# nihalsid/single-view-3d-reconstruction

Measured on AMD Instinct MI355X. Metric: query-points/sec fwd+bwd (128^3 grid, 50k pts), higher is better.
Workload: dtype f32

## Files before the change

### include/svr_hip.h

```cpp
#ifndef SVR_HIP_H
#define SVR_HIP_H

#include <stdint.h>

#ifdef __cplusplus
extern "C" {
#endif

#define SVR_OK 0
#define SVR_E_BADARG (-1)
#define SVR_E_BADSHAPE (-2)
#define SVR_E_ALIGN (-3)
#define SVR_E_UNSUPPORTED (-4)
#define SVR_E_IO (-5)
#define SVR_E_NOTFOUND (-6)
#define SVR_E_INTERNAL (-7)

#define SVR_MAX_LEVELS 6

int svr_version(void);
const char *svr_last_error(void);

typedef struct svr_pull_plan {
  const uint32_t *keys;
// ... 138 lines not shown
#define SVR_LIN_FWD_F16X3 1
#define SVR_LIN_FWD_BF16X6 2
#define SVR_LIN_BWD_DATA_F32 3
#define SVR_LIN_BWD_DATA_F16X3S 4
#define SVR_LIN_BWD_DATA_BF16X3 5
#define SVR_LIN_BWD_WEIGHT_F32 6
#define SVR_LIN_BWD_WEIGHT_F16X3S 7
#define SVR_LIN_BWD_WEIGHT_BF16X3 8
#define SVR_LIN_K_NT 0
#define SVR_LIN_K_NN 1
#define SVR_LIN_K_TN 2
#define SVR_LIN_K_NT128 3
#define SVR_LIN_K_NT64 4
#define SVR_LIN_K_NT128_BWD 5
#define SVR_LIN_K_NN_X3 6
#define SVR_LIN_K_TN_TR 7
#define SVR_LIN_K_TN_PREPASS 8
#define SVR_LIN_K_NT_X6 9
#define SVR_LIN_BIAS_NONE 0
#define SVR_LIN_BIAS_KERNEL 1
#define SVR_LIN_BIAS_COLSUM_VEC 2
#define SVR_LIN_BIAS_COLSUM_SLOW 3
int svr_linear_variant(int32_t op, int64_t M, int64_t N, int64_t K, int64_t ld_a, int64_t ld_b, int64_t ld_out,
                       int64_t ld_mask, int32_t lo_a, int32_t lo_b, int32_t lo_out, int32_t lo_mask, int32_t epilogue,
                       int32_t want_bias, int32_t *kernel, int32_t *coalesced, int32_t *splits, int64_t *rows_per_split,
                       int32_t *bias_form, int32_t *status);

int svr_fc_out_fwd(const float *H, int64_t ldh, const float *w, const float *b, float *logits,
                   const int32_t *row_map, int64_t M, int64_t K, void *stream);
int64_t svr_fc_out_bwd_workspace(int64_t M, int64_t K);
int svr_fc_out_bwd(const float *H, int64_t ldh, const float *w, const float *dlogits,
                   const int32_t *row_map, float *dH, int64_t lddh, float *dw, float *db, int64_t M,
                   int64_t K, uint32_t *amax_dh, void *workspace, void *stream);

int svr_bce_logits_sum_mean(const float *logits, const float *targets, float *loss, float *dlogits,
                            int64_t B, int64_t N, float gscale, void *workspace, void *stream);
int64_t svr_bce_ordered_workspace(int64_t B);
int svr_bce_logits_sum_mean_ordered(const float *logits, const float *targets, float *loss, float *dlogits,
                                    int64_t B, int64_t N, float gscale, void *workspace, void *stream);

int svr_conv3d_pack_weight(const float *W , float *Wp_fwd, float *Wp_bwd,
                           int32_t Ci, int32_t Co, void *stream);
int svr_conv3d_unpack_wgrad(const float *dWp , float *dW ,
                            int32_t Ci, int32_t Co, void *stream);
int svr_conv3d_k3(const float *in, const float *Wp, const float *bias, float *out, int32_t B,
                  int32_t D, int32_t H, int32_t W, int32_t Ci, int32_t Co, int epilogue,
                  const float *mask, void *stream);
int64_t svr_conv3d_c1_fwd_stats_workspace(int32_t B, int32_t D, int32_t H, int32_t W, int32_t Co);
int svr_conv3d_c1_fwd_stats(const float *in, const float *Wp, const float *bias, float *out, double *stats,
                            int32_t B, int32_t D, int32_t H, int32_t W, int32_t Co, int epilogue,
                            void *workspace, void *stream);
int64_t svr_conv3d_fwd_bf16x6_workspace(int32_t Ci, int32_t Co);
int svr_conv3d_k3_fwd_bf16x6(const float *in, const float *W, const float *bias, float *out, int32_t B,
                             int32_t D, int32_t H, int32_t Wd, int32_t Ci, int32_t Co, int epilogue,
                             void *workspace, void *stream);
int64_t svr_conv3d_fwd_f16x3_workspace(int32_t Ci, int32_t Co);
int svr_conv3d_k3_fwd_f16x3(const float *in, const float *W, const float *bias, float *out, int32_t B,
                             int32_t D, int32_t H, int32_t Wd, int32_t Ci, int32_t Co, int epilogue,
                             void *workspace, void *stream);
int32_t svr_conv3d_fwd_f16x3_stats_blocks(int32_t B, int32_t D, int32_t H, int32_t Wd, int32_t Ci, int32_t Co);
int svr_conv3d_k3_fwd_f16x3_stats(const float *in, const float *W, const float *bias, float *out, double *part, int32_t B,
                                  int32_t D, int32_t H, int32_t Wd, int32_t Ci, int32_t Co, int epilogue,
                                  void *workspace, void *stream);
int64_t svr_conv3d_bwd_data_bf16x3_workspace(int32_t Ci, int32_t Co);
int svr_conv3d_k3_bwd_data_bf16x3(const float *dout, const float *W, float *din, int32_t B, int32_t D,
                                  int32_t H, int32_t Wd, int32_t Ci, int32_t Co, int epilogue,
// ... 295 lines not shown
```

### single-view-3d-reconstruction_amd/_lib.py

```python
import ctypes as C
import os

import numpy as np
import torch

_HERE = os.path.dirname(os.path.abspath(__file__))
LIB_PATH = os.path.join(_HERE, "lib", "libsvr_hip.so")

SVR_MAX_LEVELS = 6
EPI_NONE, EPI_BIAS, EPI_BIAS_RELU, EPI_MASK = 0, 1, 2, 3

P = C.c_void_p
I32, I64, F32 = C.c_int32, C.c_int64, C.c_float


class Conv2dDesc(C.Structure):
    _fields_ = [("src0", P), ("src1", P), ("B", I32), ("H", I32), ("W", I32), ("C0", I32), ("C1", I32), ("k", I32),
                ("stride", I32), ("act", I32), ("upsample", I32)]


class PullPlan(C.Structure):
    _fields_ = [("keys", P), ("recs", P), ("heads", P), ("n_items", I64)]


# ... 32 lines not shown
    "svr_gather_trilinear_fwd": (C.c_int, [C.POINTER(GatherDesc), P, P, P]),
    "svr_gather_fc0_supported": (C.c_int32, [C.POINTER(GatherDesc)]),
    "svr_gather_fc0_workspace": (C.c_int64, [C.POINTER(GatherDesc), I32]),
    "svr_gather_fc0_fwd": (C.c_int, [C.POINTER(GatherDesc), P, P, I64, P, P, I64, I32, P, I64, P, C.c_uint32, I32, P, P]),
    "svr_gather_fc0_prepare": (C.c_int, [C.POINTER(GatherDesc), P, I64, I32, P, I64, P, C.c_uint32, P, P]),
    "svr_gather_fc0_run": (C.c_int, [C.POINTER(GatherDesc), P, P, P, I64, I32, P, I64, P, C.c_uint32, I32, P, P]),
    "svr_gather_fc0_bf16_prepare": (C.c_int, [C.POINTER(GatherDesc), P, I64, I32, P, P]),
    "svr_gather_fc0_bf16_run": (C.c_int, [C.POINTER(GatherDesc), P, P, P, I64, I32, I32, P, P]),
    "svr_gather_trilinear_bwd": (C.c_int, [C.POINTER(GatherDesc), P, P, P, P]),
    "svr_gather_corner_indices": (C.c_int, [C.POINTER(GatherDesc), I32, P, P, P]),
    "svr_cast_f32_to_bf16": (C.c_int, [P, P, I64, P]),
    "svr_gather_trilinear_fwd_bf16": (C.c_int, [C.POINTER(GatherDesc), P, P, P]),
    "svr_linear_fwd_bf16": (C.c_int, [P, I64, P, I64, P, P, I64, I64, I64, I64, C.c_int, P]),
    "svr_fc_out_fwd_bf16": (C.c_int, [P, I64, P, P, P, P, I64, I64, P]),
    "svr_linear_fwd": (C.c_int, [P, I64, P, I64, P, P, I64, I64, I64, I64, C.c_int, P, I64, P]),
    "svr_linear_bwd_data": (C.c_int, [P, I64, P, I64, P, I64, I64, I64, I64, C.c_int, P, I64, P]),
    "svr_linear_bwd_weight_workspace": (I64, [I64, I64, I64]),
    "svr_linear_bwd_weight": (C.c_int, [P, I64, P, I64, P, I64, P, I64, I64, I64, P, P]),
    "svr_linear_fwd_bf16x6_workspace": (I64, [I64, I64]),
    "svr_linear_fwd_bf16x6": (C.c_int, [P, I64, P, I64, P, P, I64, I64, I64, I64, C.c_int, P, P]),
    "svr_linear_fwd_f16x3_workspace": (I64, [I64, I64]),
    "svr_linear_fwd_f16x3": (C.c_int, [P, I64, P, I64, P, P, I64, I64, I64, I64, C.c_int, P, P]),
    "svr_linear_bwd_data_bf16x3_workspace": (I64, [I64, I64]),
    "svr_linear_bwd_data_bf16x3": (C.c_int, [P, I64, P, I64, P, I64, I64, I64, I64, C.c_int, P, I64, P, P]),
    "svr_linear_bwd_weight_bf16x3_workspace": (I64, [I64, I64, I64]),
    "svr_linear_bwd_weight_bf16x3": (C.c_int, [P, I64, P, I64, P, I64, P, I64, I64, I64, P, P]),
    "svr_amax_f32": (C.c_int, [P, I64, I64, I64, P, P]),
    "svr_linear_bwd_data_f16x3_workspace": (I64, [I64, I64]),
    "svr_linear_bwd_data_f16x3": (C.c_int, [P, I64, P, I64, P, I64, I64, I64, I64, C.c_int, P, I64, P, P, P, P]),
    "svr_linear_bwd_weight_f16x3_workspace": (I64, [I64, I64, I64]),
    "svr_linear_bwd_weight_f16x3": (C.c_int, [P, I64, P, I64, P, I64, P, I64, I64, I64, P, P, P]),
    "svr_linear_variant": (C.c_int, [I32, I64, I64, I64, I64, I64, I64, I64, I32, I32, I32, I32, I32, I32, P, P, P, P, P, P]),
    "svr_fc_out_fwd": (C.c_int, [P, I64, P, P, P, P, I64, I64, P]),
    "svr_fc_out_bwd_workspace": (I64, [I64, I64]),
    "svr_fc_out_bwd": (C.c_int, [P, I64, P, P, P, P, I64, P, P, I64, I64, P, P, P]),
    "svr_bce_logits_sum_mean": (C.c_int, [P, P, P, P, I64, I64, F32, P, P]),
    "svr_bce_ordered_workspace": (I64, [I64]),
    "svr_bce_logits_sum_mean_ordered": (C.c_int, [P, P, P, P, I64, I64, F32, P, P]),
    "svr_conv3d_pack_weight": (C.c_int, [P, P, P, I32, I32, P]),
    "svr_conv3d_unpack_wgrad": (C.c_int, [P, P, I32, I32, P]),
    "svr_conv3d_k3": (C.c_int, [P, P, P, P, I32, I32, I32, I32, I32, I32, C.c_int, P, P]),
    "svr_conv3d_fwd_bf16x6_workspace": (I64, [I32, I32]),
    "svr_conv3d_k3_fwd_bf16x6": (C.c_int, [P, P, P, P, I32, I32, I32, I32, I32, I32, C.c_int, P, P]),
    "svr_conv3d_fwd_f16x3_workspace": (I64, [I32, I32]),
    "svr_conv3d_k3_fwd_f16x3": (C.c_int, [P, P, P, P, I32, I32, I32, I32, I32, I32, C.c_int, P, P]),
    "svr_conv3d_fwd_f16x3_stats_blocks": (I32, [I32, I32, I32, I32, I32, I32]),
    "svr_conv3d_k3_fwd_f16x3_stats": (C.c_int, [P, P, P, P, P, I32, I32, I32, I32, I32, I32, C.c_int, P, P]),
    "svr_conv3d_bwd_data_bf16x3_workspace": (I64, [I32, I32]),
    "svr_conv3d_k3_bwd_data_bf16x3": (C.c_int, [P, P, P, I32, I32, I32, I32, I32, I32, C.c_int, P, P, P]),
    "svr_conv3d_c1_fwd_stats_workspace": (I64, [I32, I32, I32, I32, I32]),
    "svr_conv3d_c1_fwd_stats": (C.c_int, [P, P, P, P, P, I32, I32, I32, I32, I32, C.c_int, P, P]),
    "svr_conv3d_k3_bwd_weight_workspace": (I64, [I32, I32, I32, I32, I32, I32]),
    "svr_conv3d_k3_bwd_weight": (C.c_int, [P, P, P, P, I32, I32, I32, I32, I32, I32, P, P]),
    "svr_conv3d_k3_bwd_weight_bf16x3_workspace": (I64, [I32, I32, I32, I32, I32, I32]),
    "svr_conv3d_k3_bwd_weight_bf16x3": (C.c_int, [P, P, P, P, I32, I32, I32, I32, I32, I32, P, P]),
    "svr_conv3d_k3_bwd_weight_bf16x3_param": (C.c_int, [P, P, P, P, I32, I32, I32, I32, I32, I32, P, P]),
    "svr_conv3d_bwd_data_f16x3_workspace": (I64, [I32, I32]),
    "svr_conv3d_k3_bwd_data_f16x3": (C.c_int, [P, P, P, I32, I32, I32, I32, I32, I32, C.c_int, P, P, P, P, P]),
    "svr_conv3d_k3_bwd_weight_f16x3": (C.c_int, [P, P, P, P, I32, I32, I32, I32, I32, I32, I32, P, P, P]),
    "svr_conv3d_k3_variant": (C.c_int, [I32, I32, I32, I32, I32, I32, I32, P, P, P, P, P]),
    "svr_conv3d_k3_bwd_weight_variant": (C.c_int, [I32, I32, I32, I32, I32, I32, I32, P, P, P]),
    "svr_bn_stats_workspace": (I64, [I64, I32]),
    "svr_bn_stats": (C.c_int, [P, P, I64, I32, P, P]),
    "svr_bn_stats_finalize": (C.c_int, [P, P, P, P, P, P, P, P, P, I64, I32, F32, F32, P, P]),
    "svr_bn_finalize_parts": (C.c_int, [P, I32, P, P, P, P, P, P, P, P, I64, I32, F32, F32, P]),
    "svr_bn_finalize": (C.c_int, [P, P, P, P, P, P, P, I64, I32, F32, F32, C.c_int, P]),
# ... 169 lines not shown
```

### single-view-3d-reconstruction_amd/build.py

```python
import os
import subprocess
import sys

HERE = os.path.dirname(os.path.abspath(__file__))
CSRC = os.path.join(HERE, "csrc")
INCLUDE = os.path.join(os.path.dirname(HERE), "include")
LIBDIR = os.path.join(HERE, "lib")
LIB = os.path.join(LIBDIR, "libsvr_hip.so")

SOURCES = {
    "capi.cpp": [],
    "gather.hip": ["-ffp-contract=off"],
    "gather_fc0.hip": ["-ffp-contract=off"],
    "sort.hip": [],
    "gemm.hip": [],
    "gemm_bf16x3.hip": [],
    "gemm_bf16x6.hip": [],
    "gemm_f16x3.hip": [],
    "conv3d.hip": [],
    "conv3d_bf16.hip": [],
    "conv3d_bwdw_bf16.hip": [],
    "bn_pool.hip": [],
    "stage1.hip": [],
    "projection.hip": ["-ffp-contract=off"],
    "bf16_path.hip": ["-ffp-contract=off"],
    "mesh_occupancy.hip": ["-ffp-contract=off"],
    "marching_cubes.hip": ["-ffp-contract=off"],
    "sparse_lattice.hip": ["-ffp-contract=off"],
    "voxel_mesh.hip": ["-ffp-contract=off"],
    "mesh_eval.hip": ["-ffp-contract=off"],
    "mesh_df.hip": ["-ffp-contract=off"],
    "raycast.hip": ["-ffp-contract=off"],
    "vertex_color.hip": ["-ffp-contract=off"],
    "mesh_components.hip": ["-ffp-contract=off"],
    "mesh_simplify.hip": ["-ffp-contract=off"],
    "mesh_smooth.hip": ["-ffp-contract=off"],
    "sample_io.hip": [],
    "io_npz.cpp": [],
    "io_df.cpp": [],
    "io_exr.cpp": [],
    "io_mesh.cpp": [],
    "io_png.cpp": [],
    "raw_sample.hip": ["-ffp-contract=off"],
    "conv2d.hip": [],
    "conv2d_igemm.hip": [],
    "depth_head.hip": ["-ffp-contract=off"],
    "rgb_preprocess.hip": ["-ffp-contract=off"],
}
HOST = ("capi.cpp", "io_npz.cpp", "io_df.cpp", "io_exr.cpp", "io_mesh.cpp", "io_png.cpp")
HOST_COMMON = ["-O3", "-fPIC", "-std=c++17", "-ffp-contract=off", "-I" + INCLUDE, "-I" + CSRC]
COMMON = ["-O3", "-fPIC", "--offload-arch=gfx950", "-munsafe-fp-atomics", "-std=c++17", "-I" + INCLUDE, "-I" + CSRC,
# ... 83 lines not shown
```

### single-view-3d-reconstruction_amd/model/ifnet.py

```python
import contextlib
import copy
import os

import torch
import torch.nn as nn

from .. import ops
from ..arena import StepArena

_ARCH = {
    128: dict(stages=[(("conv_in",), "conv_in_bn"), (("conv_0", "conv_0_1"), "conv0_1_bn"),
                      (("conv_1", "conv_1_1"), "conv1_1_bn"), (("conv_2", "conv_2_1"), "conv2_1_bn"),
                      (("conv_3", "conv_3_1"), "conv3_1_bn")],
              disp=0.0722, align_corners=False),
    32: dict(stages=[(("conv_1", "conv_1_1"), "conv1_1_bn"), (("conv_2", "conv_2_1"), "conv2_1_bn"),
                     (("conv_3", "conv_3_1"), "conv3_1_bn")],
             disp=0.035, align_corners=True),
}


def _displacements(d):
    rows = [[0.0, 0.0, 0.0]]
    for axis in range(3):
        for sign in (-1, 1):
# ... 467 lines not shown
                     main, gfeat.device, arena, need_pts, skip, proj, len(levels))
        dw0 = db0 = None
        if ctx.fused:
            dh0, feat, ctx.feat = gfeat, ctx.feat, None
            dw0, db0, gfeat = _fc0_kept_bwd(fork, dh0, feat, ctx.w0p, klay, arena)
            if link is not None:
                link.dh0 = dh0
        if link is not None and link.dh0 is None:
            raise RuntimeError("IF-Net HIP path: the projected backward needs dh0 from the point MLP's backward")
        gpts = _scatter_kept(fork, ext, levels, gvols, pts, gfeat, scatter_layout, orders, plans, ready, skip, proj, need_pts)
        if proj:
            dh0, link.dh0 = link.dh0, None
            dw0 = _project_wide(fork, ext, levels, gvols, pts, dh0, ctx.w0p, orders, ready, proj, dPs, dw0)
        if fork.on and not fork.pipelined:
            fork.join()
            feat = None
        grads, gx = _stages_bwd(fork, ext, saved, gvols, ctx.training, need_x)
        if need_x:
            fork.wait_level(0)
            gx = (gx + gvols[0]).view(ctx.x_shape)
        if fork.pipelined:
            fork.join()
        if lease is not None:
            lease.release()
        return (None, None, None, None, dw0, db0, gx, gpts) + tuple(grads.get(p) for p in ext._param_list)


class _PointMLPFn(torch.autograd.Function):

    @staticmethod
    def forward(ctx, feat, row_map, w0p, b0, w1, b1, w2, b2, wo, bo, link=None):
        ctx.headless = w0p is None
        h0 = feat if ctx.headless else ops.linear_fwd(feat, w0p, b0, relu=True)
        h1 = ops.linear_fwd(h0, w1, b1, relu=True)
        h2 = ops.linear_fwd(h1, w2, b2, relu=True)
        logits = ops.fc_out_fwd(h2, wo, bo, row_map)
        ctx.save_for_backward(*(() if ctx.headless else (feat, w0p)), w1, w2, wo, h0, h1, h2)
        ctx.row_map = row_map
        ctx.link = link
        return logits

    @staticmethod
    def backward(ctx, dlogits):
        *head, w1, w2, wo, h0, h1, h2 = ctx.saved_tensors
        dh2, dwo, dbo = ops.fc_out_bwd(h2, wo, dlogits.contiguous(), ctx.row_map)
        dw2, db2 = ops.linear_bwd_weight(dh2, h1)
        dh1 = ops.linear_bwd_data(dh2, w2, mask=h1)
        dw1, db1 = ops.linear_bwd_weight(dh1, h0)
        dh0 = ops.linear_bwd_data(dh1, w1, mask=h0)
        tail = (dw1, db1, dw2, db2, dwo, dbo, None)
        if ctx.headless:
            return (dh0, None, None, None) + tail
        (feat, w0p), link = head, ctx.link
        if link is None:
            dw0, db0 = ops.linear_bwd_weight(dh0, feat)
            dfeat = ops.linear_bwd_data(dh0, w0p) if ctx.needs_input_grad[0] else None
            return (dfeat, None, dw0, db0) + tail
        link.dh0 = dh0
        dw0 = torch.zeros_like(w0p)
        dfeat = torch.empty_like(feat)
        db0 = None
        for a, b in link.keep:
            dws, dbs = ops.linear_bwd_weight(dh0, feat[:, a:b], want_bias=db0 is None)
            dw0[:, a:b] = dws
            db0 = dbs if db0 is None else db0
            if (a, b) in link.raw and not link.need_level0:
                continue
            ops.linear_bwd_data(dh0, w0p[:, a:b], out=dfeat[:, a:b])
        return (dfeat, None, dw0, db0) + tail
# ... 141 lines not shown
            self.fc_0 = nn.Conv1d(feature_size, hidden_dim * 2, 1)
            self.fc_1 = nn.Conv1d(hidden_dim * 2, hidden_dim, 1)
            self.fc_2 = nn.Conv1d(hidden_dim, hidden_dim, 1)
        else:
            raise NotImplementedError(f"net_res={net_res}")
        self.fc_out = nn.Conv1d(hidden_dim, 1, 1)
        self.actvn = nn.ReLU()
        perm = self.ifnet_feature_extractor._layout.reference_permutation()
        self.register_buffer("_fc0_perm", perm, persistent=False)
        self.register_buffer("_fc0_src", perm.clamp(min=0), persistent=False)
        self.register_buffer("_fc0_mask", perm < 0, persistent=False)
        inv = torch.empty(int((perm >= 0).sum()), dtype=torch.long)
        inv[perm[perm >= 0]] = torch.nonzero(perm >= 0).squeeze(1)
        self.register_buffer("_fc0_inv", inv, persistent=False)

    def _fc0_internal(self):
        return _PermuteColumnsFn.apply(self.fc_0.weight.squeeze(2), self._fc0_src, self._fc0_mask, self._fc0_inv)

    @torch.no_grad()
    def _prepare_weights_async(self, lease):
        if not PREPARE_WEIGHTS_AHEAD:
            return
        ext = self.ifnet_feature_extractor
        prep = ext._prepared
        main, side = torch.cuda.current_stream(), _get_side_stream(self.fc_out.weight.device)
        side.wait_stream(main)
        with torch.cuda.stream(side):
            prep.begin()
            for which in ("fwd", "bwd"):
                for convs, _ in ext._stages:
                    for conv in convs:
                        if conv.weight.shape[1] > 1:
                            prep.add_conv(conv.weight.detach(), which)
                prep.add_linear(self.fc_1.weight.detach().squeeze(2), which)
                prep.add_linear(self.fc_2.weight.detach().squeeze(2), which)
                if which == "fwd":
                    prep.mark(side)
            prep.finish(side)
        ops.set_prepared(prep)

        def expire():
            prep.invalidate()
            if ops._prepared is prep:
                ops.set_prepared(None)
        lease.on_release.append(expire)

    @torch.no_grad()
    def encode(self, x, storage="f32"):
        levels = self.ifnet_feature_extractor.encode_levels(x)
        if storage == "bf16":
            return [ops.cast_bf16(v) for v in levels]
        if storage != "f32":
            raise ValueError(f"storage={storage!r}")
        return levels

    @torch.no_grad()
    def _query_bf16(self, levels, points, row_map, prepared=None):
        B, N = points.shape[0], points.shape[1]
        ext = self.ifnet_feature_extractor
        if prepared is None and FUSE_FC0_BF16 and ops.gather_fc0_bf16_supported(levels, ext._layout, ext._disp, ext._align,
                                                                                self.fc_0.out_channels):
            prepared = ops.gather_fc0_bf16_prepare(levels, ext._layout, ext._disp, ext._align, self._fc0_internal())
        if prepared is not None:
            _check_prepared_for(prepared["vols"], levels)
            h = ops.gather_fc0_bf16_run(prepared, points, self.fc_0.bias, relu=True)
        else:
            rows = ops.gather_fwd_bf16(levels, points, ext._layout, ext._disp, ext._align)
            h = ops.linear_fwd_bf16(rows, ops.cast_bf16(self._fc0_internal()), self.fc_0.bias, relu=True)
# ... 4 lines not shown
    @torch.no_grad()
    def prepare_query(self, levels, max_points):
        ext = self.ifnet_feature_extractor
        if levels[0].dtype == torch.bfloat16:
            if FUSE_FC0_BF16 and ops.gather_fc0_bf16_supported(levels, ext._layout, ext._disp, ext._align, self.fc_0.out_channels):
                return ops.gather_fc0_bf16_prepare(levels, ext._layout, ext._disp, ext._align, self._fc0_internal())
            return None
        if levels[0].dtype != torch.float32 or not FUSE_FC0 or self.fc_0.out_channels != 256:
            return None
        B = levels[0].shape[0]
        probe = torch.empty(B, 1, 3, device=levels[0].device)
        if not ops.gather_fc0_supported(levels, probe, ext._layout, ext._disp, ext._align, self.fc_0.out_channels):
            return None
        return ops.gather_fc0_prepare(levels, ext._layout, ext._disp, ext._align, self._fc0_internal(), B, int(max_points))

    @torch.no_grad()
    def query(self, levels, points, spatial_sort=False, prepared=None):
        B, N = points.shape[0], points.shape[1]
        points = points.float().contiguous()
        row_map = None
        if spatial_sort and N > 1:
            row_map, points = ops.morton_order(points, want_sorted=True)
        if levels[0].dtype == torch.bfloat16:
            return self._query_bf16(levels, points, row_map, prepared)
        ext = self.ifnet_feature_extractor
        if prepared is not None:
            _check_prepared_for(prepared.vols, levels)
            h, _ = ops.gather_fc0_run(prepared, points, self.fc_0.bias)
        elif FUSE_FC0 and ops.gather_fc0_supported(levels, points, ext._layout, ext._disp, ext._align, self.fc_0.out_channels):
            h, _ = ops.gather_fc0_fwd(levels, points, ext._layout, ext._disp, ext._align, self._fc0_internal(), self.fc_0.bias)
        else:
            rows = ext.feature_rows_from_levels(levels, points)
            h = ops.linear_fwd(rows, self._fc0_internal(), self.fc_0.bias, relu=True)
        h = ops.linear_fwd(h, self.fc_1.weight.squeeze(2), self.fc_1.bias, relu=True)
        h = ops.linear_fwd(h, self.fc_2.weight.squeeze(2), self.fc_2.bias, relu=True)
        return ops.fc_out_fwd(h, self.fc_out.weight.reshape(-1).contiguous(), self.fc_out.bias, row_map).view(B, N)

    def forward(self, x, points, spatial_sort=True):
        B, N = points.shape[0], points.shape[1]
        if not x.is_cuda:
            raise RuntimeError("IF-Net HIP path needs GPU tensors (no CPU fallback)")
        row_map = None
        ext = self.ifnet_feature_extractor
        lease = ext._arena.lease() if (USE_ARENA and torch.is_grad_enabled() and not points.requires_grad
                                       and not torch.cuda.is_current_stream_capturing()) else None
        arena = lease.arena if lease is not None else None
        ext._points_ready = None
        if spatial_sort and N > 1:
            pts = points.detach().float().contiguous()
            if arena is not None and SORT_ON_SIDE_STREAM and not os.environ.get("SVR_NO_SIDE_STREAM"):
                self._prepare_weights_async(lease)
                main, side = torch.cuda.current_stream(), _get_side_stream(x.device)
                side.wait_stream(main)
                with torch.cuda.stream(side):
                    row_map, sorted_pts = ops.morton_order(pts, want_sorted=True, arena=arena)
                    ext._points_ready = torch.cuda.Event()
                    ext._points_ready.record(side)
            else:
                row_map, sorted_pts = ops.morton_order(pts, want_sorted=True, arena=arena)
            if points.requires_grad:
                points = points.reshape(B * N, 3)[row_map.long()].view(B, N, 3)
            else:
                points = sorted_pts
        w0p = self._fc0_internal()
        link = None
        if (PROJECT_WIDE_LEVELS and torch.is_grad_enabled() and w0p.requires_grad and not points.requires_grad
                and self.fc_0.out_channels == 256 and SCATTER_FORM != "atomic"
                and not (ops.GATHER_FLAGS & ops._lib.GATHER_DETERMINISTIC)):
            wide = [l for l, c in enumerate(ext._layout.channels) if c == 128 and
# ... 91 lines not shown
```

### single-view-3d-reconstruction_amd/ops.py

```python
import ctypes as C
import os

import torch

from . import _lib
from .arena import alloc as _alloc
from ._lib import EPI_BIAS, EPI_BIAS_RELU, EPI_MASK, EPI_NONE, GatherDesc, check
from ._lib import ptr as _p, stream as _stream


def _rp(t):
    if t is None:
        return None
    if not t.is_cuda:
        raise RuntimeError("svr_amd ops need GPU tensors (the HIP path has no CPU fallback)")
    return t.data_ptr()


def _f32(*ts):
    for t in ts:
        if t is not None and t.dtype != torch.float32:
            raise RuntimeError(f"expected float32, got {t.dtype}")


# ... 486 lines not shown
            ws = self._buf(("cb", w.data_ptr()), l.svr_conv3d_bwd_data_bf16x3_workspace(Ci, Co), w.device)
            check(l.svr_conv3d_k3_bwd_data_bf16x3(z, _p(w), z, 0, 0, 0, 0, Ci, Co, EPI_NONE, z, _p(ws), _stream()),
                  "conv3d_bwd_data_bf16x3 prepare")
            self._valid[("cb", w.data_ptr())] = (w._version, len(self._events))
        if bwd and BACKWARD_CONV == "f16x3s" and Ci % 2 == 0 and Co % 16 == 0:
            ws = self._buf(("cbh", w.data_ptr()), l.svr_conv3d_bwd_data_f16x3_workspace(Ci, Co), w.device)
            check(l.svr_conv3d_k3_bwd_data_f16x3(z, _p(w), z, 0, 0, 0, 0, Ci, Co, EPI_NONE, z, z, z, _p(ws), _stream()),
                  "conv3d_bwd_data_f16x3 prepare")
            self._valid[("cbh", w.data_ptr())] = (w._version, len(self._events))

    def add_linear(self, w, which="both"):
        _f32(w)
        N, K = w.shape
        assert w.stride(1) == 1
        l = _lib.lib()
        z = C.c_void_p(0)
        fwd, bwd = which in ("fwd", "both"), which in ("bwd", "both")
        if fwd and FORWARD_GEMM == "f16x3" and K % 16 == 0:
            ws = self._buf(("lf", w.data_ptr()), l.svr_linear_fwd_f16x3_workspace(N, K), w.device)
            check(l.svr_linear_fwd_f16x3(z, 0, C.c_void_p(w.data_ptr()), w.stride(0), z, z, 0, 0, N, K, EPI_NONE, _p(ws), _stream()),
                  "linear_fwd_f16x3 prepare")
            self._valid[("lf", w.data_ptr())] = (w._version, len(self._events))
        if bwd and BACKWARD_GEMM == "bf16x3" and N % 32 == 0 and K % 4 == 0:
            ws = self._buf(("lb", w.data_ptr()), l.svr_linear_bwd_data_bf16x3_workspace(N, K), w.device)
            check(l.svr_linear_bwd_data_bf16x3(z, 0, C.c_void_p(w.data_ptr()), w.stride(0), z, 0, 0, N, K, EPI_NONE, z, 0, _p(ws),
                                               _stream()), "linear_bwd_data_bf16x3 prepare")
            self._valid[("lb", w.data_ptr())] = (w._version, len(self._events))
        if bwd and BACKWARD_GEMM == "f16x3s" and N % 16 == 0:
            ws = self._buf(("lbh", w.data_ptr()), l.svr_linear_bwd_data_f16x3_workspace(N, K), w.device)
            check(l.svr_linear_bwd_data_f16x3(z, 0, C.c_void_p(w.data_ptr()), w.stride(0), z, 0, 0, N, K, EPI_NONE, z, 0, z, z,
                                              _p(ws), _stream()), "linear_bwd_data_f16x3 prepare")
            self._valid[("lbh", w.data_ptr())] = (w._version, len(self._events))

    def mark(self, stream):
        ev = torch.cuda.Event()
        ev.record(stream)
        self._events.append(ev)

    def finish(self, stream):
        self.mark(stream)
        self.ready = self._events[-1]

    def invalidate(self):
        self._valid.clear()

    def lookup(self, kind, w):
        key = (kind, w.data_ptr())
        ver, idx = self._valid.get(key, (-1, 0))
        if ver != w._version or idx >= len(self._events):
            return None
        cur = torch.cuda.current_stream()
        if (idx, cur.cuda_stream) not in self._waited:
            cur.wait_event(self._events[idx])
            self._waited.add((idx, cur.cuda_stream))
        return self._ws[key]


_prepared = None


def set_prepared(p):
    global _prepared
    _prepared = p


def _lookup(kind, w, mode, default):
    if _prepared is None or (mode is not None and mode != default):
        return None
    return _prepared.lookup(kind, w)


LINEAR_OPS = {"fwd_f32": 0, "fwd_f16x3": 1, "fwd_bf16x6": 2, "bwd_data_f32": 3, "bwd_data_f16x3s": 4, "bwd_data_bf16x3": 5,
              "bwd_weight_f32": 6, "bwd_weight_f16x3s": 7, "bwd_weight_bf16x3": 8}
LINEAR_KERNELS = ("nt", "nn", "tn", "nt128", "nt64", "nt128_bwd", "nn_x3", "tn_tr", "tn_prepass", "nt_x6")
LINEAR_BIAS_FORMS = ("none", "kernel", "colsum_vec", "colsum_slow")


def operand_layout(t):
    return None if t is None else (t.stride(0), t.data_ptr() & 15, t.stride(1) == 1)


def _al16(lay):
    return lay is None or (lay[2] and lay[0] % 4 == 0 and lay[1] == 0)


def _linear_fwd_op(mode, K):
    mode = mode or FORWARD_GEMM
    return "fwd_" + mode if mode in ("f16x3", "bf16x6") and K % 16 == 0 else "fwd_f32"


def _linear_bwd_data_op(mode, N, dy, out, mask):
    mode = mode or BACKWARD_GEMM
    if mode == "f16x3s":
        return "bwd_data_f16x3s" if N % 16 == 0 and _al16(dy) and _al16(out) and _al16(mask) else "bwd_data_f32"
    if mode == "bf16x3" and N % 32 == 0 and out[1] == 0 and (mask is None or mask[1] == 0):
        return "bwd_data_bf16x3"
    return "bwd_data_f32"


def _linear_bwd_weight_op(mode, M, N, K, dy, x):
    mode = mode or BACKWARD_GEMM
    if mode == "f16x3s":
        return "bwd_weight_f16x3s" if N % 4 == 0 and K % 4 == 0 and N >= 4 and K >= 4 and M > 0 and _al16(dy) and _al16(x) else "bwd_weight_f32"
    return "bwd_weight_bf16x3" if mode == "bf16x3" and N % 4 == 0 else "bwd_weight_f32"


def linear_variant(kind, mode, M, N, K, a=None, b=None, out=None, mask=None, epilogue=None, want_bias=False):
    cont = {"fwd": (K, K, N), "bwd_data": (N, K, K), "bwd_weight": (N, K, K)}[kind]
    a, b, out = [(ld, 0, True) if lay is None else lay for lay, ld in zip((a, b, out), cont)]
    if kind == "fwd":
        op = _linear_fwd_op(mode, K)
    elif kind == "bwd_data":
        op = _linear_bwd_data_op(mode, N, a, out, mask)
    else:
        op = _linear_bwd_weight_op(mode, M, N, K, a, b)
    if epilogue is None:
        epilogue = EPI_MASK if mask is not None else EPI_NONE
    m = mask if mask is not None else (0, 0, True)
    i32 = [C.c_int32() for _ in range(5)]
    rows = C.c_int64()
    kernel, coalesced, splits, bias, status = i32
# ... 5 lines not shown


def linear_fwd(x, w, bias, relu=True, out=None, mode=None):
    _f32(x, w, bias)
    M, K = x.shape
    N = w.shape[0]
    assert w.shape[1] == K and x.stride(1) == 1 and w.stride(1) == 1
    if out is None:
        out = torch.empty(M, N, device=x.device, dtype=torch.float32)
    _f32(out)
    amax_forget(out)
    assert out.shape == (M, N) and out.stride(1) == 1
    epi = EPI_NONE if bias is None else (EPI_BIAS_RELU if relu else EPI_BIAS)
    op = _linear_fwd_op(mode, K)
    if op == "fwd_f16x3":
        l = _lib.lib()
        ws = _lookup("lf", w, mode, "f16x3") if w.stride(0) == K else None
        wptr = C.c_void_p(0) if ws is not None else C.c_void_p(w.data_ptr())
        if ws is None:
            ws = torch.empty(l.svr_linear_fwd_f16x3_workspace(N, K), device=x.device, dtype=torch.uint8)
        check(l.svr_linear_fwd_f16x3(C.c_void_p(x.data_ptr()), x.stride(0), wptr, w.stride(0), _p(bias),
                                     _rp(out), out.stride(0), M, N, K, epi, _p(ws), _stream()), "linear_fwd_f16x3")
        return out
    if op == "fwd_bf16x6":
        l = _lib.lib()
        ws = torch.empty(l.svr_linear_fwd_bf16x6_workspace(N, K), device=x.device, dtype=torch.uint8)
        check(l.svr_linear_fwd_bf16x6(C.c_void_p(x.data_ptr()), x.stride(0), C.c_void_p(w.data_ptr()), w.stride(0), _p(bias),
                                      _rp(out), out.stride(0), M, N, K, epi, _p(ws), _stream()), "linear_fwd_bf16x6")
        return out
    check(_lib.lib().svr_linear_fwd(C.c_void_p(x.data_ptr()), x.stride(0), C.c_void_p(w.data_ptr()), w.stride(0),
                                    _p(bias), _rp(out), out.stride(0), M, N, K, epi, C.c_void_p(0), 0, _stream()),
          "linear_fwd")
    return out


BACKWARD_MODES = ("bf16x3", "f16x3s", "f32")
BACKWARD_GEMM = os.environ.get("SVR_BACKWARD", "f16x3s")
if BACKWARD_GEMM not in BACKWARD_MODES:
    raise ValueError(f"SVR_BACKWARD={BACKWARD_GEMM!r}: one of {BACKWARD_MODES}")


class _AmaxSlots:
    N = 512

    def __init__(self):
        self._rings = {}

    def take(self, device):
        if torch.cuda.is_current_stream_capturing():
            return torch.zeros(1, device=device, dtype=torch.int32)
        key = (device, torch.cuda.current_stream(device).cuda_stream)
        r = self._rings.get(key)
        if r is None:
            r = self._rings[key] = {"buf": torch.zeros(self.N, device=device, dtype=torch.int32), "i": 0}
        i = r["i"]
        if i % (self.N // 2) == 0 and (i or r.get("lap")):
            r["buf"][i:i + self.N // 2].zero_()
        r["i"] = (i + 1) % self.N
        if r["i"] == 0:
            r["lap"] = True
        r["serial"] = r.get("serial", 0) + 1
        w = r["buf"][i:i + 1]
        w._svr_ring, w._svr_serial = r, r["serial"]
        return w

    @staticmethod
# ... 915 lines not shown
```

Before: 26.08 million.

## Fuse fc_1, fc_2 and fc_out forward into one MFMA kernel

Adds a single HIP kernel that runs both 256-wide hidden linear layers and the output projection for a 64-row tile, keeping the intermediate activations in LDS as split f16 hi/lo planes and streaming h1/h2 out only for backward. Weights are pre-split into fragment-ordered f16x3 planes during the existing weight-prep pass and prefetched in a rotating 4-stage register ring. This removes two kernel launches and the global round trips of re-reading h1 and h2 between layers, and the model's forward paths now call it. In exchange it uses large LDS and register footprints (two workgroups per CU) and only applies to hidden size 256 with f16x3 forward mode.

```diff
diff --git a/include/svr_hip.h b/include/svr_hip.h
--- a/include/svr_hip.h
+++ b/include/svr_hip.h
@@ -194,6 +194,11 @@
 int svr_fc_out_bwd(const float *H, int64_t ldh, const float *w, const float *dlogits,
                    const int32_t *row_map, float *dH, int64_t lddh, float *dw, float *db, int64_t M,
                    int64_t K, uint32_t *amax_dh, void *workspace, void *stream);
+
+int64_t svr_mlp_tail_fwd_workspace(int64_t hidden);
+int svr_mlp_tail_fwd(const float *h0, int64_t ldh0, const float *W1, const float *b1, const float *W2, const float *b2,
+                     const float *w_out, const float *b_out, float *h1, int64_t ldh1, float *h2, int64_t ldh2,
+                     float *logits, const int32_t *row_map, int64_t M, int64_t hidden, void *workspace, void *stream);
 
 int svr_bce_logits_sum_mean(const float *logits, const float *targets, float *loss, float *dlogits,
                             int64_t B, int64_t N, float gscale, void *workspace, void *stream);
diff --git a/single-view-3d-reconstruction_amd/_lib.py b/single-view-3d-reconstruction_amd/_lib.py
--- a/single-view-3d-reconstruction_amd/_lib.py
+++ b/single-view-3d-reconstruction_amd/_lib.py
@@ -88,6 +88,8 @@
     "svr_linear_bwd_weight_f16x3": (C.c_int, [P, I64, P, I64, P, I64, P, I64, I64, I64, P, P, P]),
     "svr_linear_variant": (C.c_int, [I32, I64, I64, I64, I64, I64, I64, I64, I32, I32, I32, I32, I32, I32, P, P, P, P, P, P]),
     "svr_fc_out_fwd": (C.c_int, [P, I64, P, P, P, P, I64, I64, P]),
+    "svr_mlp_tail_fwd_workspace": (I64, [I64]),
+    "svr_mlp_tail_fwd": (C.c_int, [P, I64, P, P, P, P, P, P, P, I64, P, I64, P, P, I64, I64, P, P]),
     "svr_fc_out_bwd_workspace": (I64, [I64, I64]),
     "svr_fc_out_bwd": (C.c_int, [P, I64, P, P, P, P, I64, P, P, I64, I64, P, P, P]),
     "svr_bce_logits_sum_mean": (C.c_int, [P, P, P, P, I64, I64, F32, P, P]),
diff --git a/single-view-3d-reconstruction_amd/build.py b/single-view-3d-reconstruction_amd/build.py
--- a/single-view-3d-reconstruction_amd/build.py
+++ b/single-view-3d-reconstruction_amd/build.py
@@ -17,6 +17,7 @@
     "gemm_bf16x3.hip": [],
     "gemm_bf16x6.hip": [],
     "gemm_f16x3.hip": [],
+    "mlp_tail.hip": [],
     "conv3d.hip": [],
     "conv3d_bf16.hip": [],
     "conv3d_bwdw_bf16.hip": [],
diff --git a/single-view-3d-reconstruction_amd/csrc/mlp_tail.hip b/single-view-3d-reconstruction_amd/csrc/mlp_tail.hip
--- /dev/null
+++ b/single-view-3d-reconstruction_amd/csrc/mlp_tail.hip
@@ -0,0 +1,235 @@
+#include "common.h"
+#include "f16x3.h"
+#include "mlp_tail_layout.h"
+
+using namespace svr;
+
+namespace {
+
+constexpr int TH = (int)kMlpTailHidden;
+constexpr int TTM = 64;
+constexpr int TNW = 8;
+constexpr int TJT = TH / (32 * TNW);
+constexpr int TNT = 64 * TNW;
+constexpr int TRW = TTM / TNW;
+constexpr int TLW = 8;
+constexpr int TNK = TH / 16;
+constexpr int TPLANE = TTM * TLW;
+constexpr int TKSTEP = 2 * TPLANE + 8;
+constexpr int T_LDS_BYTES = TNK * TKSTEP * 4;
+constexpr int WKSTEP = 2 * (TH / 32) * 512;
+static_assert((TNW == 4 || TNW == 8) && TH == 256 && T_LDS_BYTES >= TTM * TH * 4 && 2 * T_LDS_BYTES <= 160 * 1024, "the f32 h2 tile fits; two workgroups per CU");
+
+__device__ __forceinline__ int wfrag_index(int kk, int plane, int n) {
+  return ((((kk >> 4) * 2 + plane) * (TH / 32) + (n >> 5)) * 64 + ((kk >> 3) & 1) * 32 + (n & 31)) * 8 + (kk & 7);
+}
+
+__global__ __launch_bounds__(64) void mlp_tail_split_w_kernel(const float *__restrict__ W, int64_t ldw, const uint32_t *__restrict__ amax,
+                                                              uint16_t *__restrict__ p0) {
+  const int kk = blockIdx.x * 64 + threadIdx.x, n = blockIdx.y;
+  const float w = W[(int64_t)n * ldw + kk] * w_scale(amax[0], false);
+  _Float16 h, l;
+  split_w(w, h, l);
+  p0[wfrag_index(kk, 0, n)] = __builtin_bit_cast(uint16_t, h);
+  p0[wfrag_index(kk, 1, n)] = __builtin_bit_cast(uint16_t, l);
+}
+
+__device__ __forceinline__ float lane_xor1(float v) {
+  return __int_as_float(__builtin_amdgcn_mov_dpp(__float_as_int(v), 0xB1, 0xf, 0xf, true));
+}
+
+__global__ __launch_bounds__(TNT, TNW / 2) void mlp_tail_kernel(const float *__restrict__ H0, int64_t ldh0, const uint16_t *__restrict__ P1,
+                                                          const uint32_t *__restrict__ amax1, const float *__restrict__ b1,
+                                                          const uint16_t *__restrict__ P2, const uint32_t *__restrict__ amax2,
+                                                          const float *__restrict__ b2, const float *__restrict__ wo,
+                                                          const float *__restrict__ bo, float *__restrict__ H1, int64_t ldh1,
+                                                          float *__restrict__ H2, int64_t ldh2, float *__restrict__ logits,
+                                                          const int32_t *__restrict__ row_map, int64_t M) {
+  extern __shared__ __attribute__((aligned(16))) uint32_t lds[];
+  const int t = threadIdx.x, lane = t & 63, wc = t >> 6;
+  const int l31 = lane & 31, lh = lane >> 5;
+  const int64_t m0 = (int64_t)blockIdx.x * TTM;
+
+  uint4 w[4][TJT][2];
+  const int woff = ((TJT * wc) * 64 + lane) * 8;
+  auto loadb = [&](uint4 (&r)[TJT][2], int g) {
+    const uint16_t *q = (g < TNK ? P1 + g * WKSTEP : P2 + (g - TNK) * WKSTEP) + woff;
+#pragma unroll
+    for (int jt = 0; jt < TJT; ++jt) {
+      r[jt][0] = *reinterpret_cast<const uint4 *>(q + jt * 512);
+      r[jt][1] = *reinterpret_cast<const uint4 *>(q + (TH / 32) * 512 + jt * 512);
+    }
+  };
+#pragma unroll
+  for (int g = 0; g < 3; ++g) loadb(w[g], g);
+
+  {
+    float4 x[TRW];
+#pragma unroll
+    for (int i = 0; i < TRW; ++i) {
+      int64_t m = m0 + wc * TRW + i;
+      m = m < M ? m : M - 1;
+      x[i] = *reinterpret_cast<const float4 *>(H0 + m * ldh0 + lane * 4);
+    }
+#pragma unroll
+    for (int i = 0; i < TRW; ++i) {
+      uint32_t h0, l0, h1, l1;
+      split_x(x[i].x, x[i].y, h0, l0);
+      split_x(x[i].z, x[i].w, h1, l1);
+      const int off = (lane >> 2) * TKSTEP + slot_dw(wc * TRW + i, (lane & 3) >> 1) + (lane & 1) * 2;
+      *reinterpret_cast<uint2 *>(lds + off) = make_uint2(h0, h1);
+      *reinterpret_cast<uint2 *>(lds + TPLANE + off) = make_uint2(l0, l1);
+    }
+  }
+  __syncthreads();
+
+  f32x16 acc[2][TJT];
+  auto layer = [&](int g0) {
+#pragma unroll
+    for (int i = 0; i < 2; ++i)
+#pragma unroll
+      for (int jt = 0; jt < TJT; ++jt)
+#pragma unroll
+        for (int r = 0; r < 16; ++r) acc[i][jt][r] = 0.f;
+#pragma unroll
+    for (int ks = 0; ks < TNK; ++ks) {
+      const int g = g0 + ks;
+      if (g + 3 < 2 * TNK) loadb(w[(g + 3) & 3], g + 3);
+      const uint4(&cur)[TJT][2] = w[g & 3];
+      f16x8 b[3][TJT];
+#pragma unroll
+      for (int jt = 0; jt < TJT; ++jt) {
+        union { uint4 q; f16x8 v; } u0, u1;
+        u0.q = cur[jt][0];
+        u1.q = cur[jt][1];
+        b[0][jt] = u0.v;
+        b[1][jt] = u1.v;
+        b[2][jt] = scale_2m11(u0.v);
+      }
+      const uint32_t *pa = lds + ks * TKSTEP;
+#pragma unroll
+      for (int i = 0; i < 2; ++i) {
+        const f16x8 ah = frag_f16(pa + slot_dw(i * 32 + l31, lh)), al = frag_f16(pa + TPLANE + slot_dw(i * 32 + l31, lh));
+#pragma unroll
+        for (int jt = 0; jt < TJT; ++jt) {
+          acc[i][jt] = __builtin_amdgcn_mfma_f32_32x32x16_f16(al, b[2][jt], acc[i][jt], 0, 0, 0);
+          acc[i][jt] = __builtin_amdgcn_mfma_f32_32x32x16_f16(ah, b[1][jt], acc[i][jt], 0, 0, 0);
+          acc[i][jt] = __builtin_amdgcn_mfma_f32_32x32x16_f16(ah, b[0][jt], acc[i][jt], 0, 0, 0);
+        }
+      }
+    }
+  };
+
+  layer(0);
+  __syncthreads();
+  {
+    const float inv = w_scale(amax1[0], true);
+    const int odd = l31 & 1;
+#pragma unroll
+    for (int i = 0; i < 2; ++i)
+#pragma unroll
+      for (int jt = 0; jt < TJT; ++jt) {
+        const int n = 32 * TJT * wc + jt * 32 + l31, c = n & ~1;
+        const float bv = b1[n];
+        const int koff = (c >> 4) * TKSTEP + ((c & 7) >> 1), sub = (c & 15) >> 3;
+#pragma unroll
+        for (int p = 0; p < 8; ++p) {
+          const int row = i * 32 + ((2 * p) & 3) + 8 * ((2 * p) >> 2) + 4 * lh;
+          const float v0 = fmaxf(acc[i][jt][2 * p] * inv + bv, 0.f), v1 = fmaxf(acc[i][jt][2 * p + 1] * inv + bv, 0.f);
+          if (m0 + row < M) __builtin_nontemporal_store(v0, H1 + (m0 + row) * ldh1 + n);
+          if (m0 + row + 1 < M) __builtin_nontemporal_store(v1, H1 + (m0 + row + 1) * ldh1 + n);
+          const float got = lane_xor1(odd ? v0 : v1);
+          uint32_t hi, lo;
+          split_x(odd ? got : v0, odd ? v1 : got, hi, lo);
+          const int off = koff + slot_dw(row + odd, sub);
+          lds[off] = hi;
+          lds[TPLANE + off] = lo;
+        }
+      }
+  }
+  __syncthreads();
+
+  layer(TNK);
+  __syncthreads();
+  float *ct = reinterpret_cast<float *>(lds);
+  {
+    const float inv = w_scale(amax2[0], true);
+#pragma unroll
+    for (int i = 0; i < 2; ++i)
+#pragma unroll
+      for (int jt = 0; jt < TJT; ++jt) {
+        const int n = 32 * TJT * wc + jt * 32 + l31;
+        const float bv = b2[n];
+#pragma unroll
+        for (int r = 0; r < 16; ++r)
+          ct[(i * 32 + (r & 3) + 8 * (r >> 2) + 4 * lh) * TH + n] = fmaxf(acc[i][jt][r] * inv + bv, 0.f);
+      }
+  }
+  __syncthreads();
+
+  const int sub = t & 15;
+  float4 c4[4];
+#pragma unroll
+  for (int j = 0; j < 4; ++j) c4[j] = *reinterpret_cast<const float4 *>(wo + sub * 4 + 64 * j);
+#pragma unroll
+  for (int pass = 0; pass < TTM * 16 / TNT; ++pass) {
+#pragma clang fp contract(off)
+    const int row = (t >> 4) + (TNT / 16) * pass;
+    const int64_t m = m0 + row;
+    float s = 0.f;
+    if (m < M) {
+#pragma unroll
+      for (int j = 0; j < 4; ++j) {
+        const float4 a = *reinterpret_cast<const float4 *>(ct + row * TH + sub * 4 + 64 * j);
+        const float4 c = c4[j];
+        __builtin_nontemporal_store(f32x4{a.x, a.y, a.z, a.w}, reinterpret_cast<f32x4 *>(H2 + m * ldh2 + sub * 4 + 64 * j));
+        s += a.x * c.x + a.y * c.y + a.z * c.z + a.w * c.w;
+      }
+    }
+#pragma unroll
+    for (int o = 8; o >= 1; o >>= 1) s += __shfl_xor(s, o);
+    if (m < M && sub == 0) logits[row_map ? (int64_t)row_map[m] : m] = s + bo[0];
+  }
+}
+
+bool al16(const void *p, int64_t ld) { return ((uintptr_t)p & 15) == 0 && ld % 4 == 0 && ld >= TH; }
+
+}
+
+extern "C" int64_t svr_mlp_tail_fwd_workspace(int64_t hidden) {
+  if (hidden != kMlpTailHidden) return SVR_E_UNSUPPORTED;
+  return ws_measure(mlp_tail_layout, hidden);
+}
+
+extern "C" int svr_mlp_tail_fwd(const float *h0, int64_t ldh0, const float *W1, const float *b1, const float *W2, const float *b2,
+                                const float *w_out, const float *b_out, float *h1, int64_t ldh1, float *h2, int64_t ldh2,
+                                float *logits, const int32_t *row_map, int64_t M, int64_t hidden, void *workspace, void *stream) {
+  SVR_CHECK(hidden == kMlpTailHidden, SVR_E_UNSUPPORTED, "mlp_tail_fwd: hidden %ld (the kernel is built for %ld)", (long)hidden,
+            (long)kMlpTailHidden);
+  SVR_CHECK((h0 || W1) && (!W1 == !W2) && workspace, SVR_E_BADARG, "mlp_tail_fwd: null pointer");
+  if (h0 && M > 0) {
+    SVR_CHECK(b1 && b2 && w_out && b_out && h1 && h2 && logits, SVR_E_BADARG, "mlp_tail_fwd: null pointer");
+    SVR_CHECK(al16(h0, ldh0) && al16(h1, ldh1) && al16(h2, ldh2) && ((uintptr_t)w_out & 15) == 0, SVR_E_UNSUPPORTED,
+              "mlp_tail_fwd: rows must be 16-byte aligned, leading dimensions multiples of 4 (ldh0=%ld ldh1=%ld ldh2=%ld)", (long)ldh0,
+              (long)ldh1, (long)ldh2);
+  }
+  hipStream_t s = (hipStream_t)stream;
+  WsCursor c(workspace);
+  const MlpTailWs ws = mlp_tail_layout(c, hidden);
+  if (W1) {
+    const float *W[2] = {W1, W2};
+    for (int l = 0; l < 2; ++l) {
+      w_amax_launch(W[l], hidden, hidden, hidden, ws.amax[l], s);
+      hipLaunchKernelGGL(mlp_tail_split_w_kernel, dim3(TH / 64, TH), dim3(64), 0, s, W[l], hidden, ws.amax[l], ws.planes[l]);
+    }
+  }
+  if (!h0) return launch_status("mlp_tail_fwd (prepare)");
+  if (M <= 0) return launch_status("mlp_tail_fwd");
+  static const hipError_t lds_attr =
+      hipFuncSetAttribute((const void *)mlp_tail_kernel, hipFuncAttributeMaxDynamicSharedMemorySize, T_LDS_BYTES);
+  SVR_CHECK(lds_attr == hipSuccess, (int)lds_attr, "mlp_tail_fwd: cannot reserve %d bytes of LDS: %s", T_LDS_BYTES,
+            hipGetErrorString(lds_attr));
+  hipLaunchKernelGGL(mlp_tail_kernel, dim3((unsigned)cdiv(M, TTM)), dim3(TNT), T_LDS_BYTES, s, h0, ldh0, ws.planes[0], ws.amax[0], b1,
+                     ws.planes[1], ws.amax[1], b2, w_out, b_out, h1, ldh1, h2, ldh2, logits, row_map, M);
+  return launch_status("mlp_tail_fwd");
+}
diff --git a/single-view-3d-reconstruction_amd/csrc/mlp_tail_layout.h b/single-view-3d-reconstruction_amd/csrc/mlp_tail_layout.h
--- /dev/null
+++ b/single-view-3d-reconstruction_amd/csrc/mlp_tail_layout.h
@@ -0,0 +1,13 @@
+#pragma once
+#include "workspace.h"
+
+namespace svr {
+constexpr int64_t kMlpTailHidden = 256;
+struct MlpTailWs {
+  uint32_t *amax[2];
+  uint16_t *planes[2];
+};
+inline MlpTailWs mlp_tail_layout(WsCursor &c, int64_t hidden) {
+  return {{c.take<uint32_t>(64), c.take<uint32_t>(64)}, {c.take<uint16_t>(2 * hidden * hidden), c.take<uint16_t>(2 * hidden * hidden)}};
+}
+}
diff --git a/single-view-3d-reconstruction_amd/model/ifnet.py b/single-view-3d-reconstruction_amd/model/ifnet.py
--- a/single-view-3d-reconstruction_amd/model/ifnet.py
+++ b/single-view-3d-reconstruction_amd/model/ifnet.py
@@ -523,9 +523,7 @@
     def forward(ctx, feat, row_map, w0p, b0, w1, b1, w2, b2, wo, bo, link=None):
         ctx.headless = w0p is None
         h0 = feat if ctx.headless else ops.linear_fwd(feat, w0p, b0, relu=True)
-        h1 = ops.linear_fwd(h0, w1, b1, relu=True)
-        h2 = ops.linear_fwd(h1, w2, b2, relu=True)
-        logits = ops.fc_out_fwd(h2, wo, bo, row_map)
+        h1, h2, logits = ops.mlp_tail_fwd(h0, w1, b1, w2, b2, wo, bo, row_map)
         ctx.save_for_backward(*(() if ctx.headless else (feat, w0p)), w1, w2, wo, h0, h1, h2)
         ctx.row_map = row_map
         ctx.link = link
@@ -733,8 +731,10 @@
                     for conv in convs:
                         if conv.weight.shape[1] > 1:
                             prep.add_conv(conv.weight.detach(), which)
-                prep.add_linear(self.fc_1.weight.detach().squeeze(2), which)
-                prep.add_linear(self.fc_2.weight.detach().squeeze(2), which)
+                w1, w2 = self.fc_1.weight.detach().squeeze(2), self.fc_2.weight.detach().squeeze(2)
+                if which == "bwd" or not prep.add_mlp_tail(w1, w2):
+                    prep.add_linear(w1, which)
+                    prep.add_linear(w2, which)
                 if which == "fwd":
                     prep.mark(side)
             prep.finish(side)
@@ -805,9 +805,9 @@
         else:
             rows = ext.feature_rows_from_levels(levels, points)
             h = ops.linear_fwd(rows, self._fc0_internal(), self.fc_0.bias, relu=True)
-        h = ops.linear_fwd(h, self.fc_1.weight.squeeze(2), self.fc_1.bias, relu=True)
-        h = ops.linear_fwd(h, self.fc_2.weight.squeeze(2), self.fc_2.bias, relu=True)
-        return ops.fc_out_fwd(h, self.fc_out.weight.reshape(-1).contiguous(), self.fc_out.bias, row_map).view(B, N)
+        _, _, logits = ops.mlp_tail_fwd(h, self.fc_1.weight.squeeze(2), self.fc_1.bias, self.fc_2.weight.squeeze(2), self.fc_2.bias,
+                                        self.fc_out.weight.reshape(-1).contiguous(), self.fc_out.bias, row_map)
+        return logits.view(B, N)
 
     def forward(self, x, points, spatial_sort=True):
         B, N = points.shape[0], points.shape[1]
diff --git a/single-view-3d-reconstruction_amd/ops.py b/single-view-3d-reconstruction_amd/ops.py
--- a/single-view-3d-reconstruction_amd/ops.py
+++ b/single-view-3d-reconstruction_amd/ops.py
@@ -542,6 +542,21 @@
                                               _p(ws), _stream()), "linear_bwd_data_f16x3 prepare")
             self._valid[("lbh", w.data_ptr())] = (w._version, len(self._events))
 
+    def add_mlp_tail(self, w1, w2):
+        _f32(w1, w2)
+        hidden = w1.shape[1]
+        if _mlp_tail_op(None, hidden, w1, w2, None, None) != "mlp_tail_f16x3":
+            return False
+        l = _lib.lib()
+        z = C.c_void_p(0)
+        ws = self._buf(("mt", w1.data_ptr()), l.svr_mlp_tail_fwd_workspace(hidden), w1.device)
+        check(l.svr_mlp_tail_fwd(z, 0, C.c_void_p(w1.data_ptr()), z, C.c_void_p(w2.data_ptr()), z, z, z, z, 0, z, 0, z, z, 0, hidden,
+                                 _p(ws), _stream()), "mlp_tail_fwd prepare")
+        self._ws[("mt2", w2.data_ptr())] = ws
+        self._valid[("mt", w1.data_ptr())] = (w1._version, len(self._events))
+        self._valid[("mt2", w2.data_ptr())] = (w2._version, len(self._events))
+        return True
+
     def mark(self, stream):
         ev = torch.cuda.Event()
         ev.record(stream)
@@ -597,6 +612,18 @@
 def _linear_fwd_op(mode, K):
     mode = mode or FORWARD_GEMM
     return "fwd_" + mode if mode in ("f16x3", "bf16x6") and K % 16 == 0 else "fwd_f32"
+
+
+MLP_TAIL_HIDDEN = 256
+
+
+def _mlp_tail_op(mode, hidden, w1, w2, wo, h0):
+    mode = mode or FORWARD_GEMM
+    if (mode == "f16x3" and hidden == MLP_TAIL_HIDDEN and tuple(w1.shape) == (hidden, hidden) and tuple(w2.shape) == (hidden, hidden)
+            and w1.is_contiguous() and w2.is_contiguous() and (wo is None or (wo.is_contiguous() and wo.data_ptr() % 16 == 0))
+            and _al16(h0)):
+        return "mlp_tail_f16x3"
+    return "three_ops"
 
 
 def _linear_bwd_data_op(mode, N, dy, out, mask):
@@ -668,6 +695,30 @@
                                     _p(bias), _rp(out), out.stride(0), M, N, K, epi, C.c_void_p(0), 0, _stream()),
           "linear_fwd")
     return out
+
+
+def mlp_tail_fwd(h0, w1, b1, w2, b2, wo, bo, row_map=None):
+    _f32(h0, w1, b1, w2, b2, wo, bo)
+    M, K = h0.shape
+    assert w1.shape == (w1.shape[0], K) and w2.shape == (w2.shape[0], w1.shape[0]) and h0.stride(1) == 1
+    if _mlp_tail_op(None, K, w1, w2, wo, operand_layout(h0)) != "mlp_tail_f16x3":
+        h1 = linear_fwd(h0, w1, b1, relu=True)
+        h2 = linear_fwd(h1, w2, b2, relu=True)
+        return h1, h2, fc_out_fwd(h2, wo, bo, row_map)
+    l = _lib.lib()
+    h1 = torch.empty(M, K, device=h0.device, dtype=torch.float32)
+    h2 = torch.empty(M, K, device=h0.device, dtype=torch.float32)
+    logits = torch.empty(M, device=h0.device, dtype=torch.float32)
+    ws = _lookup("mt", w1, None, "f16x3")
+    if ws is not None and _lookup("mt2", w2, None, "f16x3") is not ws:
+        ws = None
+    z = C.c_void_p(0)
+    wp1, wp2 = (z, z) if ws is not None else (C.c_void_p(w1.data_ptr()), C.c_void_p(w2.data_ptr()))
+    if ws is None:
+        ws = torch.empty(l.svr_mlp_tail_fwd_workspace(K), device=h0.device, dtype=torch.uint8)
+    check(l.svr_mlp_tail_fwd(C.c_void_p(h0.data_ptr()), h0.stride(0), wp1, _p(b1), wp2, _p(b2), _p(wo), _p(bo), _p(h1), K, _p(h2), K,
+                             _p(logits), _p(row_map), M, K, _p(ws), _stream()), "mlp_tail_fwd")
+    return h1, h2, logits
 
 
 BACKWARD_MODES = ("bf16x3", "f16x3s", "f32")
```

Measured after the change: 26.42 million (median of 6 runs). +1.3%, better.
